# sb17v/GaussianK-SGD

Hardware: AMD Instinct MI355X
Metric: images/sec (whole node) ResNet-50 k=0.1% at 1/2/4/8 MI355X; effective grad compression ratio (higher is better)
Workload: dtype fp32; 1 GPU; model=resnet50, global_batch=512, per_gpu_batch=512, image_size=224, parallelism=dp1, compressor=gaussian, buckets=1, threshold=524288000, planner=threshold, exchange=local, momentum_correction=True, hip_graph=False, f32_matmul=bf16x6

## Files before the change

gaussiank_sgd_amd/ops/conv1x1.py:

```python
from __future__ import annotations

import os
from typing import Callable, Dict, List, Tuple

import torch
import torch.nn as nn
import torch.nn.functional as F

from . import load
from . import streams
from . import weight_prep

_CL = torch.channels_last
_TUNE = os.environ.get("GKSGD_GEMM_TUNE", "1") != "0"
_ENABLED = os.environ.get("GKSGD_FASTCONV", "1") != "0"
_choices: Dict[tuple, tuple] = {}
_OWN = ("hip", "w3", "mat", "wino", "wx6")
_GK_MARGIN = float(os.environ.get("GKSGD_GK_MARGIN", "0.05"))
_BIAS_COLSUM = os.environ.get("GKSGD_CONV_BIAS_COLSUM", "1") != "0"
_timings: Dict[tuple, list] = {}
_WINO = os.environ.get("GKSGD_WINO", "1") != "0"
_FORCE = os.environ.get("GKSGD_CONV_FORCE", "")
_WINO_GRIDS = (0, 1 << 20)
_NT_CFGS = [1, 2, 3, 4, 11, 13, 21, 22, 23, 24, 111, 113, 121, 122, 123, 124, 25, 26, 27, 125, 126, 127,
            211, 212, 213, 214, 221, 222, 223, 224]
_NT_GRIDS = (0, 512, 1 << 20)
_TN_CFGS = [(c, s) for c in (1, 2, 3, 4, 5, 6, 7, 8, 21, 22, 23, 24, 27, 9, 29, 101, 121, 102, 122) for s in (0, 128)]
_NT_CFGS_F32 = [1, 2, 3, 4, 7, 11, 12, 13, 14, 21, 22, 23, 24, 101, 102, 103, 104, 201, 202, 203, 204,
                1001, 1002, 1003, 1004, 1005, 1006, 1007, 1021, 1022, 1101, 1102, 1103]
_TN_CFGS_F32 = [(c, s) for c in (1, 2, 3, 4, 5, 6, 7, 8, 9, 11, 12, 13, 14, 15, 16) for s in (0, 64)]
_TN_SMALL_M = 1 << 17
_TN_SMALL_F32 = [(c, s) for c in (4, 5, 11, 14, 15) for s in (16, 32, 128)]


X6 = 100000
_NT_CFGS_X6 = [c + X6 for c in (1, 2, 3, 4, 5, 6, 7, 12, 13, 101, 102, 103, 104, 105, 106, 107, 202, 203, 1001, 1002, 1003)]
_NT_CFGS_X62 = [2 * X6 + t for t in range(1, 8)] + [3 * X6 + t for t in range(1, 8)]
_F32MM = os.environ.get("GKSGD_F32_MATMUL", "bf16x6")


def set_f32_matmul(mode: str) -> str:
    global _F32MM
    if mode not in ("native", "bf16x6"):
        raise ValueError("f32 matmul mode must be 'native' or 'bf16x6', got %r" % (mode,))
    prev, _F32MM = _F32MM, mode
    return prev


def f32_matmul() -> str:
    return _F32MM


def _x6() -> bool:
    return _F32MM == "bf16x6"


_TN_CFGS_X62 = [(2 * X6 + t, sp) for t in (1, 2, 3, 4, 5, 6, 7, 8) for sp in (0, 64)]


def _tn_cfgs(dt: torch.dtype) -> List[Tuple[int, int]]:
    if dt == torch.float32:
# ... 249 lines not shown


def _lz_kw(lz, rows: bool = False) -> dict:
    _, x, coef, padz, padx = lz
    return dict(lz_x=_rows(x) if rows else x, lz_coef=coef, lz_padz=padz, lz_padx=padx)


def _dgrad(dy: torch.Tensor, w: torch.Tensor, x_shape, s: int, lz=None, plink=None, wp: bool = False) -> torch.Tensor:
    N, C, H, W, K, k, p, OH, OW = _geom(x_shape, w, s)
    g = _g()
    dt = dy.dtype
    xs = torch.empty(x_shape, dtype=dt, device=dy.device, memory_format=_CL)
    kw = _lz_kw(lz, rows=(s == 1 and k == 1)) if lz is not None else {}

    def miopen():
        return torch.ops.aten.convolution_backward(dy, xs, w, None, [s, s], [p, p], [1, 1], False, [0, 0], 1,
                                                   [True, False, False])[0]
    cands = []
    split = []
    dx = None
    if s == 2:
        dx = xs
        z = _zero(dy.device)
        run = lambda c, mb: g.conv_dgrad_s2(dy, w, dx, z, c, mb, **kw)
        cands = [(("hip", c, mb), (lambda c=c, mb=mb: run(c, mb))) for c in _nt_cfgs(dt) for mb in _NT_GRIDS]
    if s == 1:
        dx = xs
        if k == 1:
            DY, DX = _rows(dy), _rows(dx)
            Wt = _lazy(lambda: weight_prep.transposed_1x1(w, wp))
            run = lambda c, mb: g.gemm_nt(DY, Wt(), DX, c, mb, **kw)
            if lz is None:
                split = _splitk_cfgs(dt, N * H * W, C, K)
        else:
            wf = _lazy(lambda: weight_prep.flipped_3x3(w, wp))
            z = _zero(dy.device)
            run = lambda c, mb: g.conv_nt(dy, wf(), dx, z, 1, p, c, mb, **kw)
        cands = [(("hip", c, mb), (lambda c=c, mb=mb: run(c, mb))) for c in _nt_cfgs(dt) for mb in _NT_GRIDS]
        cands += [(("hip", c, mb), (lambda c=c, mb=mb: run(c, mb))) for c in split for mb in _SPLITK_GRIDS]
    if lz is not None:
        cands.append((("mat", 0, 0), lambda: _dgrad(plink.materialize(), w, x_shape, s, wp=wp)))
        ch = _pick(("dgrad", N, C, H, W, K, k, s) + _dkey(dt) + ("lz",), cands)
        if ch[0] == "mat":
            return _dgrad(plink.materialize(), w, x_shape, s, wp=wp)
        run(ch[1], ch[2])
        return dx
    wino = _wino_ok(dt, k, s, K, C) and _wino_shape_fits(N, H, W, C, K)
    if wino:
# ... 8 lines not shown
    run(ch[1], ch[2])
    return dx


_WGRAD_AFTER = os.environ.get("GKSGD_WGRAD_AFTER_DGRAD", "0") == "1"
_SIDE_QROUNDS = int(os.environ.get("GKSGD_WGRAD_SIDE_QROUNDS", "0"))
_FORK_BIAS = os.environ.get("GKSGD_WGRAD_STREAM_BIAS", "0") == "1"
_FORKABLE = tuple(k for k in os.environ.get("GKSGD_WGRAD_STREAM_KINDS", "hip,w3,wino").split(",")
                  if k and (k != "wino" or os.environ.get("GKSGD_WGRAD_STREAM_WINO", "1") == "1"))


def _lazy(make):
    box = []

    def get():
        if not box:
            box.append(make())
        return box[0]
    return get


def _dgrad_key(N, C, H, W, K, k, s, dt) -> tuple:
    wino = _wino_ok(dt, k, s, K, C) and _wino_shape_fits(N, H, W, C, K)
    return ("dgrad", N, C, H, W, K, k, s) + _dkey(dt) + (_wino_tag(K, C) if wino else ())


def _dgrad_bn(dy: torch.Tensor, w: torch.Tensor, x_shape, s: int, link, lz=None, plink=None,
              wp: bool = False) -> torch.Tensor:
    N, C, H, W, K, k, p, OH, OW = _geom(x_shape, w, s)
    kw = _lz_kw(lz, rows=(k == 1)) if lz is not None else {}
    g = _g()
    M = N * H * W
    dt = dy.dtype
    dz = torch.empty(x_shape, dtype=dt, device=dy.device, memory_format=_CL)
    st = torch.empty(2, min(1280, (M + 63) // 64), C, dtype=torch.float32, device=dy.device)
    h, mask, dy2 = link.h, link.mask, link.dy2
    if k == 1:
        DY, DZ = _rows(dy), _rows(dz)
        Wt = _lazy(lambda: weight_prep.transposed_1x1(w, wp))
        H2 = _rows(h)
        D2 = _rows(dy2) if dy2 is not None else None
        run = lambda c, mb: g.gemm_nt(DY, Wt(), DZ, c, mb, st, None, H2, D2, mask, **kw)
        split = _splitk_cfgs(dt, M, C, K) if lz is None else []
    else:
        split = []
        wf = _lazy(lambda: weight_prep.flipped_3x3(w, wp))
        z = _zero(dy.device)
# ... 288 lines not shown
```

gaussiank_sgd_amd/ops/csrc/bindings.cpp:

```cpp
#include <ATen/ATen.h>
#include <c10/core/DeviceGuard.h>
#include <c10/hip/HIPStream.h>
#include <torch/custom_class.h>
#include <torch/library.h>

#include <cstring>
#include <vector>

#include "comm/rccl_engine.h"
#include "kernels/gk_kernels.h"

namespace {

hipStream_t cur_stream(const at::Tensor& t) {
  return c10::hip::getCurrentHIPStream(t.device().index()).stream();
}

void check_dev(const at::Tensor& t, const char* name) {
  TORCH_CHECK(t.is_cuda(), name, " must be a GPU tensor");
  TORCH_CHECK(t.is_contiguous(), name, " must be contiguous");
}

void check_f32(const at::Tensor& t, const char* name) {
  check_dev(t, name);
// ... 1324 lines not shown
void wino_wgrad(at::Tensor x, at::Tensor dy, at::Tensor out, at::Tensor part, int64_t splits) {
  auto cl = [](const at::Tensor& t) {
    return t.is_cuda() && t.scalar_type() == at::kFloat && t.dim() == 4 && t.is_contiguous(at::MemoryFormat::ChannelsLast);
  };
  TORCH_CHECK(cl(x) && cl(dy) && cl(out), "wino_wgrad: x, dy, out must be channels-last fp32 GPU tensors");
  const int64_t N = x.size(0), C = x.size(1), H = x.size(2), W = x.size(3), K = dy.size(1);
  TORCH_CHECK(dy.size(0) == N && dy.size(2) == H && dy.size(3) == W, "wino_wgrad: dy must be [N, K, H, W]");
  TORCH_CHECK(out.size(0) == K && out.size(1) == C && out.size(2) == 3 && out.size(3) == 3,
              "wino_wgrad: out must be [K, C, 3, 3]");
  TORCH_CHECK(C % 64 == 0 && K % 64 == 0, "wino_wgrad: C and K must be multiples of 64");
  TORCH_CHECK(N * ((H + 1) / 2) * ((W + 1) / 2) < (int64_t(1) << 31) && x.numel() * 4 < (int64_t(1) << 31) &&
                  dy.numel() * 4 < (int64_t(1) << 31),
              "wino_wgrad: size out of range (x, dy bytes < 2^31: buffer-descriptor addressing)");
  TORCH_CHECK(part.is_cuda() && part.scalar_type() == at::kFloat && part.is_contiguous() &&
                  part.numel() >= wino_wgrad_ws(N, H, W, C, K, splits),
              "wino_wgrad: workspace too small (wino_wgrad_ws)");
  c10::DeviceGuard guard(x.device());
  gk::wino_wgrad(x.data_ptr<float>(), dy.data_ptr<float>(), part.data_ptr<float>(), out.data_ptr<float>(), (int)N,
                 (int)H, (int)W, (int)C, (int)K, (int)splits, cur_stream(x));
}

void conv_dgrad_s2(at::Tensor dy, at::Tensor w, at::Tensor dx, at::Tensor zero, int64_t cfg, int64_t max_blocks,
                   c10::optional<at::Tensor> lz_x, c10::optional<at::Tensor> lz_coef,
                c10::optional<at::Tensor> lz_padz, c10::optional<at::Tensor> lz_padx) {
  TORCH_CHECK(dy.is_cuda() && is_gemm_dtype(dy) && dy.dim() == 4 && dy.is_contiguous(at::MemoryFormat::ChannelsLast),
              "conv_dgrad_s2: dy must be channels-last bf16 or fp32");
  TORCH_CHECK(w.is_cuda() && w.scalar_type() == dy.scalar_type() && w.dim() == 4 && w.size(0) == dy.size(1) &&
                  w.size(2) == w.size(3) && (w.size(2) == 1 || w.size(2) == 3),
              "conv_dgrad_s2: w must be [K, C, k, k] of dy's dtype, k in {1, 3}");
  TORCH_CHECK(dx.is_cuda() && dx.scalar_type() == dy.scalar_type() && dx.dim() == 4 && dx.size(0) == dy.size(0) &&
                  dx.size(1) == w.size(1) && dx.is_contiguous(at::MemoryFormat::ChannelsLast),
              "conv_dgrad_s2: dx must be channels-last [N, C, H, W] of dy's dtype");
  const bool f32 = dy.scalar_type() == at::kFloat;
  const int64_t N = dy.size(0), K = dy.size(1), OHd = dy.size(2), OWd = dy.size(3);
  const int64_t C = w.size(1), k = w.size(2), H = dx.size(2), W = dx.size(3);
  const int64_t p = k / 2;
  TORCH_CHECK((H + 2 * p - k) / 2 + 1 == OHd && (W + 2 * p - k) / 2 + 1 == OWd, "conv_dgrad_s2: shape mismatch");
  TORCH_CHECK(K % 64 == 0 && C % 64 == 0, "conv_dgrad_s2: channels must be multiples of 64");
  check_zero(zero);
  TORCH_CHECK(N * H * W < (int64_t(1) << 31), "conv_dgrad_s2: too many pixels");
  gk::LazyArgs lzv{};
  const gk::LazyArgs* lz = lazy_args(lz_x, lz_coef, lz_padz, lz_padx, dy, K, &lzv) ? &lzv : nullptr;
  c10::DeviceGuard guard(dy.device());
  const hipStream_t st = cur_stream(dy);
  if (k == 1) {
    const at::Tensor wt = w.reshape({K, C}).t().contiguous();
    const int r = gk::conv_nt_remap(dy.data_ptr(), K, zero.data_ptr(), (int)OHd, (int)OWd, (int)K, (int)OHd,
                                    (int)OWd, 1, 1, wt.data_ptr(), dx.data_ptr(), N * OHd * OWd, (int)C, (int)H, (int)W,
                                    0, 0, 1, f32, (int)cfg, (int)max_blocks, lz, st);
    TORCH_CHECK(r >= 0, "conv_dgrad_s2: the lazy operand's coefficient table does not fit this tile configuration");
    return;
  }
  const at::Tensor wt = w.permute({1, 2, 3, 0}).contiguous();
  for (int a = 0; a < 2; ++a) {
    for (int b = 0; b < 2; ++b) {
      const int64_t OHc = (H - a + 1) / 2, OWc = (W - b + 1) / 2;
      if (OHc <= 0 || OWc <= 0) continue;
      at::Tensor wc = a == 0 ? wt.slice(1, 1, 2) : wt.slice(1, 0, 3, 2).flip({1});
      wc = b == 0 ? wc.slice(2, 1, 2) : wc.slice(2, 0, 3, 2).flip({2});
      wc = wc.contiguous();
      const int r = gk::conv_nt_remap(dy.data_ptr(), K, zero.data_ptr(), (int)OHd, (int)OWd, (int)K, (int)OHc,
                                      (int)OWc, a == 0 ? 1 : 2, b == 0 ? 1 : 2, wc.data_ptr(), dx.data_ptr(),
                                      N * OHc * OWc, (int)C, (int)H, (int)W, a, b, 0, f32, (int)cfg, (int)max_blocks,
                                      lz, st);
      TORCH_CHECK(r >= 0, "conv_dgrad_s2: the lazy operand's coefficient table does not fit this tile configuration");
    }
  }
}

int64_t wgrad3_ws(int64_t N, int64_t H, int64_t W, int64_t C, int64_t K) {
  return gk::wgrad3_ws_floats((int)N, (int)H, (int)W, (int)C, (int)K);
}

void conv3_wgrad(at::Tensor dy, at::Tensor x, at::Tensor out, at::Tensor part, at::Tensor zero) {
  TORCH_CHECK(x.is_cuda() && x.scalar_type() == at::kBFloat16 && x.dim() == 4 &&
                  x.is_contiguous(at::MemoryFormat::ChannelsLast),
              "conv3_wgrad: x must be channels-last bf16 [N, C, H, W]");
  const int64_t N = x.size(0), C = x.size(1), H = x.size(2), W = x.size(3);
  TORCH_CHECK(dy.is_cuda() && dy.scalar_type() == at::kBFloat16 && dy.dim() == 4 && dy.size(0) == N &&
                  dy.size(2) == H && dy.size(3) == W && dy.is_contiguous(at::MemoryFormat::ChannelsLast),
              "conv3_wgrad: dy must be channels-last bf16 [N, K, H, W]");
  const int64_t K = dy.size(1);
  TORCH_CHECK(gk::wgrad3_supported((int)H, (int)W, (int)C, (int)K), "conv3_wgrad: unsupported shape");
  TORCH_CHECK(N * H * W < (int64_t(1) << 31), "conv3_wgrad: too many pixels");
  TORCH_CHECK(out.is_cuda() && out.scalar_type() == at::kFloat && out.dim() == 4 && out.size(0) == K &&
                  out.size(1) == C && out.size(2) == 3 && out.size(3) == 3,
              "conv3_wgrad: out must be fp32 [K, C, 3, 3]");
  TORCH_CHECK(part.is_cuda() && part.scalar_type() == at::kFloat && part.is_contiguous() &&
// ... 528 lines not shown
  m.def("stem_wgrad(Tensor x, Tensor dy, Tensor(a!) out, Tensor(b!) part) -> ()");
  m.def("stem_f32_supported(int H, int W) -> bool", [](int64_t H, int64_t W) { return gk::stem_f32_supported((int)H, (int)W); });
  m.def("stem_f32_fwd(Tensor x, Tensor w, Tensor(a!) y, Tensor(b!)? stats=None) -> int");
  m.def("stem_f32x6_wplanes() -> int", &stem_f32x6_wplanes);
  m.def("stem_f32x6_fwd(Tensor x, Tensor w, Tensor(a!) y, Tensor(b!)? stats, Tensor(c!) wp3) -> int");
  m.def("stem_f32_wgrad_ws(int N) -> int", &stem_f32_wgrad_ws);
  m.def("stem_f32_wgrad(Tensor x, Tensor dy, Tensor(a!) out, Tensor(b!) part, bool x6=False) -> ()");
  m.def("wgrad3_supported(int H, int W, int C, int K) -> bool", [](int64_t H, int64_t W, int64_t C, int64_t K) {
    return gk::wgrad3_supported((int)H, (int)W, (int)C, (int)K);
  });
  m.def("wgrad3_ws(int N, int H, int W, int C, int K) -> int", &wgrad3_ws);
  m.def("conv3_wgrad(Tensor dy, Tensor x, Tensor(a!) out, Tensor(b!) part, Tensor zero) -> ()");
  m.def("wino_weights(Tensor w, Tensor(a!) u, bool flip) -> ()");
  m.def("weight_prep(Tensor table, int ndesc, int total_blocks) -> ()");
  m.def("weight_prep_blocks(int kind, int R, int S) -> int", &weight_prep_blocks);
  m.def("wino_wgrad_ws(int N, int H, int W, int C, int K, int splits=0) -> int", &wino_wgrad_ws);
  m.def("wino_wgrad(Tensor x, Tensor dy, Tensor(a!) out, Tensor(b!) part, int splits=0) -> ()");
  m.def("wino_conv(Tensor x, Tensor u, Tensor(a!) y, int max_blocks=0, Tensor(b!)? stats=None, Tensor? bn_h=None, "
        "Tensor? bn_dy2=None, Tensor? bn_mask=None, int splits=1) -> int");
  m.def("wino_x6_weights(Tensor w, Tensor(a!) u3, bool flip) -> ()");
  m.def("wino_x6_conv(Tensor x, Tensor u3, Tensor(a!) y, int max_blocks=0, Tensor(b!)? stats=None, "
        "Tensor? bn_h=None, Tensor? bn_dy2=None, Tensor? bn_mask=None) -> int");
  m.def("conv_dgrad_s2(Tensor dy, Tensor w, Tensor(a!) dx, Tensor zero, int cfg=0, int max_blocks=0, "
        "Tensor? lz_x=None, Tensor? lz_coef=None, Tensor? lz_padz=None, Tensor? lz_padx=None) -> ()");
  m.def("bn_bwd_lazy_pre(Tensor x, Tensor part, int rows, Tensor? w, Tensor mean, Tensor invstd, "
        "Tensor(a!) dgamma, Tensor(b!) dbeta, Tensor(c!) coef, Tensor(d!) padz, Tensor(e!) padx, "
        "Tensor(f!)? gw_acc=None, Tensor(g!)? gb_acc=None) -> ()");
  m.def("bn_act_backward_lazy(Tensor dy, Tensor? dy2, Tensor? mask, Tensor x, Tensor(a!) dz, Tensor? w, "
        "Tensor mean, Tensor invstd, Tensor(b!) dgamma, Tensor(c!) dbeta, Tensor(d!) ws, bool relu, "
        "Tensor(e!) coef, Tensor(f!) padz, Tensor(g!) padx, Tensor(h!)? gw_acc=None, Tensor(i!)? gb_acc=None) -> ()");
  m.def("bn_lazy_apply(Tensor dz, Tensor x, Tensor(a!) dx, Tensor coef) -> ()");
  m.def("bn_stats_partials(Tensor x, Tensor(a!) ws) -> ()");
  m.def(
      "bn_act_backward_pre_dual(Tensor dz, Tensor x, Tensor(a!) dx, Tensor? w, Tensor mean, Tensor invstd, "
      "Tensor(b!) dgamma, Tensor(c!) dbeta, Tensor part, int rows, Tensor(d!)? gw_acc, Tensor(e!)? gb_acc, Tensor x2, "
      "Tensor(f!) dx2, Tensor? w2, Tensor mean2, Tensor invstd2, Tensor(g!) dgamma2, Tensor(h!) dbeta2, "
      "Tensor(i!) ws2, Tensor(j!)? gw2_acc, Tensor(k!)? gb2_acc) -> ()");
  m.def("bn_act_backward_pre(Tensor dz, Tensor x, Tensor(a!) dx, Tensor? w, Tensor mean, Tensor invstd, "
        "Tensor(b!) dgamma, Tensor(c!) dbeta, Tensor part, int rows, Tensor(d!)? gw_acc=None, "
        "Tensor(e!)? gb_acc=None, Tensor(f!)? fin=None) -> ()");
  m.def("bn_fin_state_bytes(int C) -> int", &bn_fin_state_bytes);
  m.def("attn_supported(int T, int D) -> bool",
        [](int64_t T, int64_t D) { return gk::attn_supported((int)T, (int)D); });
  m.def("attn_fwd(Tensor qkv, Tensor(a!) out, Tensor(b!) lse, int heads, float p, int seed, Tensor? seed_dev=None) -> ()");
  m.def("attn_bwd(Tensor qkv, Tensor out, Tensor dout, Tensor lse, Tensor(a!) delta, Tensor(b!) dqkv, int heads, "
        "float p, int seed, Tensor? seed_dev=None) -> ()");
  m.def("attn_dropout_mask(Tensor(a!) mask, int B, int heads, int T, float p, int seed, Tensor? seed_dev=None) -> ()");
// ... 128 lines not shown
```

gaussiank_sgd_amd/ops/csrc/kernels/gemm.hip:

```cpp
#include "gemm_kern.h"

namespace gk {

static int nt_unit_b16(bool gather, GK_NT_UNIT_ARGS) {
  return gather ? nt_b16_gat(GK_NT_UNIT_PASS) : nt_b16_row(GK_NT_UNIT_PASS);
}

static int nt_unit_f32(bool gather, GK_NT_UNIT_ARGS) {
  const int fam = (cfg / 100000) % 10;
  if (fam == 2 || fam == 3) {
    if (lza || geo.KZ > 1 || geo.RH || (fam == 3) != (geo.b3 != nullptr)) return -2;
    if (gather) {
      const int64_t nimg = M / ((int64_t)geo.OH * geo.OW);
      if (geo.C % 32 != 0 || nimg * geo.H * geo.W * geo.C >= ((int64_t)1 << 31)) return -2;
      return nt_x62_gat(static_cast<const float*>(A), static_cast<const float*>(B), static_cast<float*>(C), M, N, K,
                        cfg % 100000, max_blocks, geo, stats, stats_ld, stats_rows, bb, stream);
    }
    return nt_x62_row(static_cast<const float*>(A), lda, static_cast<const float*>(B), ldb, static_cast<float*>(C),
                      ldc, M, N, K, cfg % 100000, max_blocks, geo.bias, stats, stats_ld, stats_rows, bb, geo.b3, stream);
  }
  const bool x6 = (cfg / 100000) % 10 == 1;
  cfg %= 100000;
  if (x6) return gather ? nt_x6_gat(GK_NT_UNIT_PASS) : nt_x6_row(GK_NT_UNIT_PASS);
  return gather ? nt_f32_gat(GK_NT_UNIT_PASS) : nt_f32_row(GK_NT_UNIT_PASS);
}

static int tn_unit_f32x(bool gather, const float* G, int64_t ldg, const float* X, int64_t ldx, float* W, int64_t ldw,
                        int64_t M, int N, int K, int cfg, int splits, const ConvGeo& geo, const LazyArgs* lza,
                        hipStream_t stream) {
  const int fam = (cfg / 100000) % 10;
  if (fam == 3) return -2;
  if (fam == 2) {
    if (gather || lza) return -2;
    tn_x62_row(G, ldg, X, ldx, W, ldw, M, N, K, cfg % 100000, splits, stream);
  } else if (fam == 1) {
    tn_unit_x6(gather, G, ldg, X, ldx, W, ldw, M, N, K, cfg % 100000, splits, geo, lza, stream);
  } else {
    tn_unit_f32(gather, G, ldg, X, ldx, W, ldw, M, N, K, cfg % 100000, splits, geo, lza, stream);
  }
  return 0;
}

// ... 129 lines not shown
  ConvGeo g{zero, H, W, C, OH, OW, S, P, KW, bias};
  g.b3 = static_cast<const uint16_t*>(b3);
  const int K = KH * KW * C;
  const int SK = (cfg / 10000) % 10;
  const int x6 = cfg / 100000 * 100000;
  if (SK > 1) {
    const int nks = K / 32;
    if (!f32 || lazy || splitk_ws == nullptr || nks % SK != 0 || C % 32 != 0) return -1;
    ConvGeo gz{zero, H, W, C, OH, OW, S, P, KW, nullptr};
    gz.KZ = SK;
    const int r = nt_unit_f32(true, X, C, B, K, splitk_ws, N, M, N, K / SK, x6 + cfg % 10000, max_blocks, gz,
                                           nullptr, 0, 0, BnBwd{}, nullptr, stream);
    if (r < 0) return r;
    return splitk_reduce(splitk_ws, SK, M, N, static_cast<float*>(Y), N, bias, stats, stats_rows, bn, stream);
  }
  const BnBwd bb = bn ? BnBwd{bn->h, bn->dy2, bn->mask} : BnBwd{};
  const int64_t sld = (int64_t)stats_rows * N;
  return f32 ? nt_unit_f32(true, X, C, B, K, Y, N, M, N, K, cfg, max_blocks, g, stats, sld, stats_rows, bb, lazy, stream)
             : nt_unit_b16(true, X, C, B, K, Y, N, M, N, K, cfg, max_blocks, g, stats, sld, stats_rows, bb, nullptr, stream);
}

int conv_nt_remap(const void* X, int64_t ldx, const void* zero, int H, int W, int C, int OH, int OW, int KH, int KW,
                  const void* B, void* Y, int64_t M, int N, int RH, int RW, int RA, int RB, int RZ, bool f32, int cfg,
                  int max_blocks, const LazyArgs* lazy, hipStream_t stream) {
  ConvGeo g{zero, H, W, C, OH, OW, 1, 0, KW, nullptr, RH, RW, RA, RB, RZ};
  const int K = KH * KW * C;
  if (KH * KW == 1) {
    return f32 ? nt_unit_f32(false, X, ldx, B, K, Y, N, M, N, K, cfg, max_blocks, g, nullptr, 0, 0, BnBwd{}, lazy, stream)
               : nt_unit_b16(false, X, ldx, B, K, Y, N, M, N, K, cfg, max_blocks, g, nullptr, 0, 0, BnBwd{}, nullptr, stream);
  }
  return f32 ? nt_unit_f32(true, X, C, B, K, Y, N, M, N, K, cfg, max_blocks, g, nullptr, 0, 0, BnBwd{}, lazy, stream)
             : nt_unit_b16(true, X, C, B, K, Y, N, M, N, K, cfg, max_blocks, g, nullptr, 0, 0, BnBwd{}, nullptr, stream);
}

int gemm_tn_acc(const void* G, int64_t ldg, const void* X, int64_t ldx, float* W, int64_t ldw, int64_t M, int N,
                 int K, bool f32, int cfg, int splits, const LazyArgs* lazy, hipStream_t stream) {
  if (f32)
    return tn_unit_f32x(false, static_cast<const float*>(G), ldg, static_cast<const float*>(X), ldx, W, ldw, M, N, K, cfg,
                           splits, ConvGeo{}, lazy, stream);
  tn_unit_b16(false, G, ldg, X, ldx, W, ldw, M, N, K, cfg, splits, ConvGeo{}, stream);
  return 0;
}

int conv_tn_acc(const void* G, const void* X, const void* zero, int H, int W_, int C, int OH, int OW, int S, int P,
                 int KH, int KW, float* Wout, int64_t M, int N, bool f32, int cfg, int splits, const LazyArgs* lazy,
                 hipStream_t stream) {
  ConvGeo g{zero, H, W_, C, OH, OW, S, P, KW, nullptr};
  const int K = KH * KW * C;
// ... 9 lines not shown
```

gaussiank_sgd_amd/ops/csrc/kernels/gemm_inst.hip:

```cpp
#include "gemm_kern.h"

#ifndef GK_GEMM_UNIT
#error "compile with -DGK_GEMM_UNIT=<unit>"
#endif

namespace gk {

#if GK_GEMM_UNIT == 0
int nt_b16_row(GK_NT_UNIT_ARGS) { return nt_dispatch<false, uint16_t>(GK_NT_UNIT_PASS); }
#elif GK_GEMM_UNIT == 1
int nt_b16_gat(GK_NT_UNIT_ARGS) { return nt_dispatch<true, uint16_t>(GK_NT_UNIT_PASS); }
#elif GK_GEMM_UNIT == 2
int nt_f32_row(GK_NT_UNIT_ARGS) { return nt_dispatch<false, float>(GK_NT_UNIT_PASS); }
#elif GK_GEMM_UNIT == 3
int nt_f32_gat(GK_NT_UNIT_ARGS) { return nt_dispatch<true, float>(GK_NT_UNIT_PASS); }
#elif GK_GEMM_UNIT == 4
void tn_unit_b16(bool gather, const void* G, int64_t ldg, const void* X, int64_t ldx, float* W, int64_t ldw, int64_t M,
                 int N, int K, int cfg, int splits, const ConvGeo& geo, hipStream_t stream) {
  if (gather) tn_dispatch<true>(G, ldg, X, ldx, W, ldw, M, N, K, cfg, splits, geo, stream);
  else tn_dispatch<false>(G, ldg, X, ldx, W, ldw, M, N, K, cfg, splits, geo, stream);
}
void tn_unit_f32(bool gather, const float* G, int64_t ldg, const float* X, int64_t ldx, float* W, int64_t ldw,
                 int64_t M, int N, int K, int cfg, int splits, const ConvGeo& geo, const LazyArgs* lza,
                 hipStream_t stream) {
  if (gather) tn_f32_dispatch<true>(G, ldg, X, ldx, W, ldw, M, N, K, cfg, splits, geo, lza, stream);
  else tn_f32_dispatch<false>(G, ldg, X, ldx, W, ldw, M, N, K, cfg, splits, geo, lza, stream);
}
#elif GK_GEMM_UNIT == 5
int nt_x6_row(GK_NT_UNIT_ARGS) { return nt_dispatch<false, float, true>(GK_NT_UNIT_PASS); }
#elif GK_GEMM_UNIT == 6
int nt_x6_gat(GK_NT_UNIT_ARGS) { return nt_dispatch<true, float, true>(GK_NT_UNIT_PASS); }
#elif GK_GEMM_UNIT == 7
void tn_unit_x6(bool gather, const float* G, int64_t ldg, const float* X, int64_t ldx, float* W, int64_t ldw,
                int64_t M, int N, int K, int cfg, int splits, const ConvGeo& geo, const LazyArgs* lza,
                hipStream_t stream) {
  if (gather) tn_f32_dispatch<true, true>(G, ldg, X, ldx, W, ldw, M, N, K, cfg, splits, geo, lza, stream);
  else tn_f32_dispatch<false, true>(G, ldg, X, ldx, W, ldw, M, N, K, cfg, splits, geo, lza, stream);
}
#elif GK_GEMM_UNIT == 8
int nt_x62_row(const float* A, int64_t lda, const float* B, int64_t ldb, float* C, int64_t ldc, int64_t M, int N, int K,
               int cfg, int max_blocks, const float* bias, float* stats, int64_t stats_ld, int stats_rows,
               const BnBwd& bb, const uint16_t* b3, hipStream_t stream) {
  ConvGeo g{};
  g.b3 = b3;
  return nt_x62_dispatch<false>(A, lda, B, ldb, C, ldc, M, N, K, cfg, max_blocks, bias, stats, stats_ld, stats_rows, bb,
                                g, stream);
}
#elif GK_GEMM_UNIT == 9
void tn_x62_row(const float* G, int64_t ldg, const float* X, int64_t ldx, float* W, int64_t ldw, int64_t M, int N,
                int K, int cfg, int splits, hipStream_t stream) {
  tn_x62_dispatch(G, ldg, X, ldx, W, ldw, M, N, K, cfg, splits, stream);
}
#elif GK_GEMM_UNIT == 10
int nt_x62_gat(const float* A, const float* B, float* C, int64_t M, int N, int K, int cfg, int max_blocks,
               const ConvGeo& geo, float* stats, int64_t stats_ld, int stats_rows, const BnBwd& bb,
               hipStream_t stream) {
  return nt_x62_dispatch<true>(A, geo.C, B, K, C, N, M, N, K, cfg, max_blocks, geo.bias, stats, stats_ld, stats_rows,
                               bb, geo, stream);
}
#else
#error "unknown GK_GEMM_UNIT"
#endif

}
```

gaussiank_sgd_amd/ops/csrc/kernels/gemm_kern.h:

```cpp
#pragma once

#ifndef GK_XCD_REMAP
#define GK_XCD_REMAP 1
#endif
#ifndef GK_X6_SCHED
#define GK_X6_SCHED 1
#endif
#ifndef GK_X6_EXP
#define GK_X6_EXP 0
#endif
#include <hip/hip_runtime.h>

#include <type_traits>

#include "common.h"
#include "gk_kernels.h"
#include "mfma_util.h"
namespace gk {

constexpr int kMaxTaps = 4;

struct ConvGeo {
  const void* zero;
  int H, W, C, OH, OW, S, P, KW;
// ... 9 lines not shown
  const uint8_t* mask;
};

struct LazyA {
  const void* x;
  const float* coef;
  const void* padz;
  const void* padx;
  int C;
};

#define GK_NT_UNIT_ARGS                                                                                      \
  const void *A, int64_t lda, const void *B, int64_t ldb, void *C, int64_t ldc, int64_t M, int N, int K, int cfg, \
      int max_blocks, const ConvGeo &geo, float *stats, int64_t stats_ld, int stats_rows, const BnBwd &bb,      \
      const LazyArgs *lza, hipStream_t stream
#define GK_NT_UNIT_PASS A, lda, B, ldb, C, ldc, M, N, K, cfg, max_blocks, geo, stats, stats_ld, stats_rows, bb, lza, stream
int nt_b16_row(GK_NT_UNIT_ARGS);
int nt_b16_gat(GK_NT_UNIT_ARGS);
int nt_f32_row(GK_NT_UNIT_ARGS);
int nt_f32_gat(GK_NT_UNIT_ARGS);
int nt_x6_row(GK_NT_UNIT_ARGS);
int nt_x6_gat(GK_NT_UNIT_ARGS);
int nt_x62_row(const float* A, int64_t lda, const float* B, int64_t ldb, float* C, int64_t ldc, int64_t M, int N, int K,
               int cfg, int max_blocks, const float* bias, float* stats, int64_t stats_ld, int stats_rows,
               const BnBwd& bb, const uint16_t* b3, hipStream_t stream);
int nt_x62_gat(const float* A, const float* B, float* C, int64_t M, int N, int K, int cfg, int max_blocks,
               const ConvGeo& geo, float* stats, int64_t stats_ld, int stats_rows, const BnBwd& bb,
               hipStream_t stream);
void tn_x62_row(const float* G, int64_t ldg, const float* X, int64_t ldx, float* W, int64_t ldw, int64_t M, int N,
                int K, int cfg, int splits, hipStream_t stream);
void tn_unit_x6(bool gather, const float* G, int64_t ldg, const float* X, int64_t ldx, float* W, int64_t ldw,
                int64_t M, int N, int K, int cfg, int splits, const ConvGeo& geo, const LazyArgs* lza,
                hipStream_t stream);
void tn_unit_b16(bool gather, const void* G, int64_t ldg, const void* X, int64_t ldx, float* W, int64_t ldw, int64_t M,
                 int N, int K, int cfg, int splits, const ConvGeo& geo, hipStream_t stream);
void tn_unit_f32(bool gather, const float* G, int64_t ldg, const float* X, int64_t ldx, float* W, int64_t ldw,
                 int64_t M, int N, int K, int cfg, int splits, const ConvGeo& geo, const LazyArgs* lza,
                 hipStream_t stream);

namespace {

__device__ __forceinline__ int swz(int r) { return (r >> 1) & 7; }

__device__ __forceinline__ void xcd_remap2(int& bx, int& by) {
  const int gx = (int)gridDim.x, gy = (int)gridDim.y, G = gx * gy;
  bx = (int)blockIdx.x;
  by = (int)blockIdx.y;
  if (!GK_XCD_REMAP || (G & 7) != 0 || G < 16) return;
// ... 505 lines not shown
      }
    }
    if (pf) stage_advance();
    st3 = st2;
    st2 = st1;
    st1 = 0;
    if (++ks == nk) {
      ks = 0;
      const int64_t mbase = mt * Cfg::BM;
      mt += gridDim.x;
      const bool full = mbase + Cfg::BM <= M;
      const bool odd = fq & 1;
#pragma unroll
      for (int ms = 0; ms < MSB; ++ms) {
        const int64_t m = mbase + wm * Cfg::WTM + ms * 16 + fr;
        const bool live = full || m < M;
        int64_t orow = m;
        int zr = 0, zc = 0;
        if (geo.RH) {
          const uint32_t ohw = (uint32_t)(geo.OH * geo.OW);
          const uint32_t mu = (uint32_t)(m < M ? m : M - 1);
          const uint32_t ni = mu / ohw, rem = mu - ni * ohw;
          const uint32_t oh = rem / (uint32_t)geo.OW, ow = rem - oh * (uint32_t)geo.OW;
          orow = ((int64_t)ni * geo.RH + 2 * oh + geo.RA) * geo.RW + 2 * ow + geo.RB;
          zr = (int)(2 * oh + 1) < geo.RH;
          zc = (int)(2 * ow + 1) < geo.RW;
        }
        if constexpr (F32) {
          f32x4 ehv[4], ed2[4];
          uint32_t ebits[4];
          if constexpr (PRE) {
            const int slot = ms % PMS;
#pragma unroll
            for (int ns = 0; ns < 4; ++ns) {
              ehv[ns] = pre_h[slot][ns];
              ed2[ns] = pre_d[slot][ns];
              ebits[ns] = pre_b[slot][ns];
            }
            if (ms + PMS < MSB) bn_row_load(mbase, ms + PMS, pre_h[slot], pre_d[slot], pre_b[slot]);
          } else if (bnb) {
#pragma unroll
            for (int ns = 0; ns < 4; ++ns) {
              ehv[ns] = ed2[ns] = f32x4{0.f, 0.f, 0.f, 0.f};
              ebits[ns] = 0u;
            }
            if (live) {
#pragma unroll
// ... 991 lines not shown
      if (pc >= 0 && pc != Cfg::PRA + p) continue;
      const int cid = tid + Cfg::THREADS * p;
      const int r = cid >> 2;
      const int off = r * 64 + (((cid & 3) ^ x62_swz(r)) << 4);
      if constexpr (P3) {
        *reinterpret_cast<u32x4*>(sb + off) = rb3[q][p][0];
        *reinterpret_cast<u32x4*>(sb + Cfg::PB + off) = rb3[q][p][1];
        *reinterpret_cast<u32x4*>(sb + 2 * Cfg::PB + off) = rb3[q][p][2];
      } else {
        bf16x8 h, m, l;
        split3x8(rb[q][p][0], rb[q][p][1], h, m, l);
        *reinterpret_cast<bf16x8*>(sb + off) = h;
        *reinterpret_cast<bf16x8*>(sb + Cfg::PB + off) = m;
        *reinterpret_cast<bf16x8*>(sb + 2 * Cfg::PB + off) = l;
      }
    }
  };

  f32x4 acc[4][4];
#pragma unroll
  for (int a = 0; a < 4; ++a)
#pragma unroll
    for (int b = 0; b < 4; ++b) acc[a][b] = f32x4{0.f, 0.f, 0.f, 0.f};
  float ssum[4][4], ssq[4][4], bia[BNB ? 1 : 4][4];
#pragma unroll
  for (int a = 0; a < 4; ++a)
#pragma unroll
    for (int b = 0; b < 4; ++b) {
      ssum[a][b] = ssq[a][b] = 0.f;
      if constexpr (!BNB) bia[a][b] = bias ? bias[n0 + wn * 64 + a * 16 + fq * 4 + b] : 0.f;
    }

  auto epilogue = [&](int64_t mt) __attribute__((always_inline)) {
    const int64_t mbase = mt * Cfg::BM;
    constexpr int EH = BNB ? 1 : 4;
#pragma unroll
    for (int ms = 0; ms < 4; ++ms) {
      const int64_t m = mbase + wm * 64 + ms * 16 + fr;
      const bool live = m < M;
#pragma unroll
      for (int nh = 0; nh < 4; nh += EH) {
      f32x4 ehv[EH], ed2[EH];
      uint32_t ebits[EH];
      if constexpr (BNB) {
#pragma unroll
        for (int e = 0; e < EH; ++e) {
          ehv[e] = ed2[e] = f32x4{0.f, 0.f, 0.f, 0.f};
          ebits[e] = 0u;
        }
        if (live) {
#pragma unroll
          for (int e = 0; e < EH; ++e) {
            const int n = n0 + wn * 64 + (nh + e) * 16 + fq * 4;
            ehv[e] = *reinterpret_cast<const f32x4*>(static_cast<const float*>(bb.h) + m * ldc + n);
            if (bb.dy2) ed2[e] = *reinterpret_cast<const f32x4*>(static_cast<const float*>(bb.dy2) + m * ldc + n);
            ebits[e] = bb.mask ? (uint32_t)bb.mask[m * (Ntot >> 2) + (n >> 2)] : 0xfu;
          }
        }
      }
#pragma unroll
      for (int e = 0; e < EH; ++e) {
        const int ns = nh + e;
// ... 1 lines not shown
        f32x4 v = acc[ms][ns];
        acc[ms][ns] = f32x4{0.f, 0.f, 0.f, 0.f};
        if constexpr (!BNB) {
#pragma unroll
          for (int r = 0; r < 4; ++r) v[r] += bia[ns][r];
        }
        if constexpr (BNB) {
#pragma unroll
          for (int r = 0; r < 4; ++r) {
            const float dz = (ebits[e] >> r) & 1u ? v[r] + ed2[e][r] : 0.f;
            v[r] = dz;
            ssum[ns][r] += dz;
            ssq[ns][r] = fmaf(dz, ehv[e][r], ssq[ns][r]);
          }
        } else {
          if (stats && live) {
#pragma unroll
            for (int r = 0; r < 4; ++r) {
              ssum[ns][r] += v[r];
              ssq[ns][r] = fmaf(v[r], v[r], ssq[ns][r]);
            }
          }
        }
        if (live) *reinterpret_cast<f32x4*>(C + m * ldc + n) = v;
      }
      }
    }
  };

  using I0 = std::integral_constant<int, 0>;
  using I1 = std::integral_constant<int, (NPF > 1 ? 1 : 0)>;
  issue_loads(I0{});
  split_write(0, I0{});
  if (T_ > 1) issue_loads(I1{});
  if (NPF > 1 && T_ > 2) issue_loads(I0{});
  __syncthreads();
  int ks = 0;
  int64_t mt = bx;
  auto slice = [&](int t, auto PAR) __attribute__((always_inline)) {
    constexpr int par = decltype(PAR)::value;
    using SN = std::integral_constant<int, (NPF > 1 ? (par ^ 1) : 0)>;
    const int cur = par;
    const char* st = smem + cur * Cfg::STAGE;
    const char* pa = st;
    const char* pb = st + 3 * Cfg::PA;
    auto frag = [&](const char* plane, int row) __attribute__((always_inline)) -> bf16x8 {
      return *reinterpret_cast<const bf16x8*>(plane + row * 64 + ((fq ^ x62_swz(row)) << 4));
    };
// ... 468 lines not shown
```

gaussiank_sgd_amd/ops/csrc/kernels/gk_kernels.h:

```cpp
#pragma once

#include <hip/hip_runtime.h>
#include <stddef.h>
#include <stdint.h>

namespace gk {

enum Mode : int {
  kModeGaussian = 0,
  kModeRedSync = 1,
  kModeRedSyncTrim = 2,
  kModeTopK = 3,
  kModeRandomK = 4,
  kModeThreshold = 5,
  kModeDGC = 6,
  kModeGaussianCal = 7,
};

constexpr int kCalFallback = 16;
constexpr int kOverflowExact = 17;

constexpr int kMaxCand = 16;
constexpr int kRecHdr = 4;
constexpr int kMaxCountBlocks = 1024;
// ... 216 lines not shown
  const uint8_t* mask;
};
struct LazyArgs {
  const void* x;
  const float* coef;
  const void* padz;
  const void* padx;
  int C;
};
int gemm_nt(const void* A, int64_t lda, const void* B, int64_t ldb, void* C, int64_t ldc, int64_t M, int N, int K,
            bool f32, int cfg, int max_blocks, float* stats, int stats_rows, const float* bias, const BnBwdArgs* bn,
            const LazyArgs* lazy, hipStream_t stream, float* splitk_ws = nullptr, const void* b3 = nullptr);
int splitk_reduce(const float* ws, int S, int64_t M, int N, float* C, int64_t ldc, const float* bias, float* stats,
                  int stats_rows, const BnBwdArgs* bn, hipStream_t stream);
int gemm_tn_acc(const void* G, int64_t ldg, const void* X, int64_t ldx, float* W, int64_t ldw, int64_t M, int N,
                 int K, bool f32, int cfg, int splits, const LazyArgs* lazy, hipStream_t stream);
int conv_nt(const void* X, const void* zero, int H, int W, int C, int OH, int OW, int S, int P, int KH, int KW,
            const void* B, void* Y, int64_t M, int N, bool f32, int cfg, int max_blocks, float* stats, int stats_rows,
            const float* bias, const BnBwdArgs* bn, const LazyArgs* lazy, hipStream_t stream,
            float* splitk_ws = nullptr, const void* b3 = nullptr);
void split3_rows(const float* src, int64_t ld, void* dst, int64_t R, int S, hipStream_t stream);
int conv_nt_remap(const void* X, int64_t ldx, const void* zero, int H, int W, int C, int OH, int OW, int KH, int KW,
                  const void* B, void* Y, int64_t M, int N, int RH, int RW, int RA, int RB, int RZ, bool f32, int cfg,
                  int max_blocks, const LazyArgs* lazy, hipStream_t stream);
int conv_tn_acc(const void* G, const void* X, const void* zero, int H, int W, int C, int OH, int OW, int S, int P,
                 int KH, int KW, float* Wout, int64_t M, int N, bool f32, int cfg, int splits, const LazyArgs* lazy,
                 hipStream_t stream);
bool stem_f32_supported(int H, int W);
int stem_f32_wgrad_blocks(int N);
int stem_f32x6_wplanes();
int stem_f32x6_forward(const float* x, int N, int H, int W, const float* w, int64_t s0, int64_t s1, int64_t s2,
                       int64_t s3, uint16_t* wp3, float* y, float* stats, int stats_rows, hipStream_t stream);
int stem_f32_forward(const float* x, int N, int H, int W, const float* w, int64_t s0, int64_t s1, int64_t s2,
                     int64_t s3, float* y, float* stats, int stats_rows, hipStream_t stream);
void stem_f32_wgrad(const float* x, const float* dy, int N, int H, int W, float* part, float* out, int64_t s0,
                    int64_t s1, int64_t s2, int64_t s3, bool x6, hipStream_t stream);
void wino_weights(const float* w, float* u, int Co, int Ci, int flip, hipStream_t stream);
enum PrepKind : int32_t { kPrepWino = 0, kPrepWinoFlip = 1, kPrepT32 = 2, kPrepT16 = 3, kPrepWinoX6 = 4,
                          kPrepWinoX6Flip = 5 };
struct PrepDesc {
  const void* src;
  void* dst;
  int64_t ld_in, ld_out;
  int64_t block_begin;
  int32_t kind, R, S, tiles_s;
};
static_assert(sizeof(PrepDesc) == 56, "PrepDesc layout is packed by ops/weight_prep.py");
// ... 91 lines not shown
```

gaussiank_sgd_amd/ops/weight_prep.py:

```python
from __future__ import annotations

import contextlib
import os
import struct
import threading
from typing import Callable, Dict, List, Optional, Tuple

import torch

KIND_WINO, KIND_WINO_FLIP, KIND_T32, KIND_T16, KIND_WINO_X6, KIND_WINO_X6_FLIP = 0, 1, 2, 3, 4, 5
_DESC = struct.Struct("<QQqqqiiii")
_MAX_DESCS = 512
_tls = threading.local()
ENABLED = os.environ.get("GKSGD_WEIGHT_PREP", "1") != "0"


def _ops():
    return torch.ops.gksgd


class _Entry:
    __slots__ = ("src", "dst", "descs", "ready")

    def __init__(self, src: torch.Tensor, dst: torch.Tensor, descs: List[tuple]):
# ... 146 lines not shown


def flipped_3x3(w: torch.Tensor, persistent: bool) -> torch.Tensor:
    K, C = w.shape[0], w.shape[1]

    def make():
        return torch.empty((C, K, 3, 3), dtype=w.dtype, device=w.device, memory_format=torch.channels_last)

    def fill(out):
        out.copy_(w.flip(2, 3).transpose(0, 1))
    p = current()
    if p is None or not persistent or w.dtype not in (torch.float32, torch.bfloat16) or \
            not w.is_contiguous(memory_format=torch.channels_last):
        out = make()
        fill(out)
        return out
    kind = KIND_T32 if w.dtype == torch.float32 else KIND_T16
    es = w.element_size()

    def descs(out):
        return [(kind, w.data_ptr() + (8 - t) * C * es, out.data_ptr() + t * K * es, 9 * C, 9 * K, K, C)
                for t in range(9)]
    return p.acquire(_key("f3", w), w, make, descs, fill)
```

Before: 5152 images/s.

## Enable bf16x6 register-staged kernels and cached class filters for stride-2 dgrad

Stride-2 dgrad can now use the register-staged bf16x6 GEMM family. The epilogue gains row remapping, using fast magic-number division, and sibling zero-fill, so those kernels accept remapped output geometry. Per-parity class filters for the 3x3 and 1x1 stride-2 weights are precomputed and cached through the weight-prep machinery, which removes the per-call permute, slice and contiguous copies. This adds more autotune candidates and a per-call bf16 presplit for family-3 configs, plus more complex epilogue indexing that could raise register pressure.

After: 5149 images/s, median of 2. No clear change (-0.0%).

```diff
diff --git a/gaussiank_sgd_amd/ops/conv1x1.py b/gaussiank_sgd_amd/ops/conv1x1.py
--- a/gaussiank_sgd_amd/ops/conv1x1.py
+++ b/gaussiank_sgd_amd/ops/conv1x1.py
@@ -37,6 +37,8 @@
 _NT_CFGS_X6 = [c + X6 for c in (1, 2, 3, 4, 5, 6, 7, 12, 13, 101, 102, 103, 104, 105, 106, 107, 202, 203, 1001, 1002, 1003)]
 _NT_CFGS_X62 = [2 * X6 + t for t in range(1, 8)] + [3 * X6 + t for t in range(1, 8)]
 _F32MM = os.environ.get("GKSGD_F32_MATMUL", "bf16x6")
+_S2_X62 = os.environ.get("GKSGD_DGRAD_S2_X62", "1") != "0"
+_S2_PREP = os.environ.get("GKSGD_DGRAD_S2_PREP", "1") != "0"
 
 
 def set_f32_matmul(mode: str) -> str:
@@ -332,8 +334,10 @@
     if s == 2:
         dx = xs
         z = _zero(dy.device)
-        run = lambda c, mb: g.conv_dgrad_s2(dy, w, dx, z, c, mb, **kw)
-        cands = [(("hip", c, mb), (lambda c=c, mb=mb: run(c, mb))) for c in _nt_cfgs(dt) for mb in _NT_GRIDS]
+        wc = _lazy(lambda: weight_prep.dgrad_s2_filters(w, wp)) if _S2_PREP else (lambda: None)
+        run = lambda c, mb: g.conv_dgrad_s2(dy, w, dx, z, c, mb, wcls=wc(), **kw)
+        cfgs = [c for c in _nt_cfgs(dt) if _S2_X62 or c not in _NT_CFGS_X62]
+        cands = [(("hip", c, mb), (lambda c=c, mb=mb: run(c, mb))) for c in cfgs for mb in _NT_GRIDS]
     if s == 1:
         dx = xs
         if k == 1:
@@ -388,7 +392,9 @@
 
 def _dgrad_key(N, C, H, W, K, k, s, dt) -> tuple:
     wino = _wino_ok(dt, k, s, K, C) and _wino_shape_fits(N, H, W, C, K)
-    return ("dgrad", N, C, H, W, K, k, s) + _dkey(dt) + (_wino_tag(K, C) if wino else ())
+    nox62 = s == 2 and not _S2_X62 and dt == torch.float32 and _x6()
+    return ("dgrad", N, C, H, W, K, k, s) + _dkey(dt) + (_wino_tag(K, C) if wino else ()) + \
+        (("nox62",) if nox62 else ())
 
 
 def _dgrad_bn(dy: torch.Tensor, w: torch.Tensor, x_shape, s: int, link, lz=None, plink=None,
diff --git a/gaussiank_sgd_amd/ops/csrc/bindings.cpp b/gaussiank_sgd_amd/ops/csrc/bindings.cpp
--- a/gaussiank_sgd_amd/ops/csrc/bindings.cpp
+++ b/gaussiank_sgd_amd/ops/csrc/bindings.cpp
@@ -1370,7 +1370,8 @@
 
 void conv_dgrad_s2(at::Tensor dy, at::Tensor w, at::Tensor dx, at::Tensor zero, int64_t cfg, int64_t max_blocks,
                    c10::optional<at::Tensor> lz_x, c10::optional<at::Tensor> lz_coef,
-                c10::optional<at::Tensor> lz_padz, c10::optional<at::Tensor> lz_padx) {
+                   c10::optional<at::Tensor> lz_padz, c10::optional<at::Tensor> lz_padx,
+                   c10::optional<at::Tensor> wcls) {
   TORCH_CHECK(dy.is_cuda() && is_gemm_dtype(dy) && dy.dim() == 4 && dy.is_contiguous(at::MemoryFormat::ChannelsLast),
               "conv_dgrad_s2: dy must be channels-last bf16 or fp32");
   TORCH_CHECK(w.is_cuda() && w.scalar_type() == dy.scalar_type() && w.dim() == 4 && w.size(0) == dy.size(1) &&
@@ -1391,27 +1392,60 @@
   const gk::LazyArgs* lz = lazy_args(lz_x, lz_coef, lz_padz, lz_padx, dy, K, &lzv) ? &lzv : nullptr;
   c10::DeviceGuard guard(dy.device());
   const hipStream_t st = cur_stream(dy);
+  if (wcls.has_value()) {
+    TORCH_CHECK(wcls->is_cuda() && wcls->scalar_type() == w.scalar_type() && wcls->is_contiguous() &&
+                    wcls->numel() == k * k * C * K,
+                "conv_dgrad_s2: wcls must hold the k * k * C * K class-filter elements of w's dtype");
+  }
+  const bool fam3 = (cfg / 100000) % 10 == 3;
+  TORCH_CHECK(!fam3 || f32, "conv_dgrad_s2: cfg family 3 takes fp32 operands");
+  auto presplit = [&](const void* wc, int64_t S) {
+    at::Tensor b3 = at::empty({C, 3 * S}, w.options().dtype(at::kBFloat16));
+    gk::split3_rows(static_cast<const float*>(wc), S, b3.data_ptr(), C, (int)S, st);
+    return b3;
+  };
+  const char* refused_x62 = "conv_dgrad_s2: the register-staged bf16x6 kernels (cfg digit 200000/300000) take no "
+                            "lazy operand or split-K";
+  const char* refused = "conv_dgrad_s2: the lazy operand's coefficient table does not fit this tile configuration";
   if (k == 1) {
-    const at::Tensor wt = w.reshape({K, C}).t().contiguous();
+    const at::Tensor wt = wcls.has_value() ? *wcls : w.reshape({K, C}).t().contiguous();
+    at::Tensor b3;
+    if (fam3) b3 = presplit(wt.data_ptr(), K);
     const int r = gk::conv_nt_remap(dy.data_ptr(), K, zero.data_ptr(), (int)OHd, (int)OWd, (int)K, (int)OHd,
                                     (int)OWd, 1, 1, wt.data_ptr(), dx.data_ptr(), N * OHd * OWd, (int)C, (int)H, (int)W,
-                                    0, 0, 1, f32, (int)cfg, (int)max_blocks, lz, st);
-    TORCH_CHECK(r >= 0, "conv_dgrad_s2: the lazy operand's coefficient table does not fit this tile configuration");
+                                    0, 0, 1, f32, (int)cfg, (int)max_blocks, lz, st,
+                                    b3.defined() ? b3.data_ptr() : nullptr);
+    TORCH_CHECK(r != -2, refused_x62);
+    TORCH_CHECK(r >= 0, refused);
     return;
   }
-  const at::Tensor wt = w.permute({1, 2, 3, 0}).contiguous();
+  at::Tensor wt;
+  if (!wcls.has_value()) wt = w.permute({1, 2, 3, 0}).contiguous();
+  int64_t woff = 0;
   for (int a = 0; a < 2; ++a) {
     for (int b = 0; b < 2; ++b) {
+      const int KHc = a == 0 ? 1 : 2, KWc = b == 0 ? 1 : 2;
+      const int64_t wn = (int64_t)KHc * KWc * C * K;
+      const int64_t wo = woff;
+      woff += wn;
       const int64_t OHc = (H - a + 1) / 2, OWc = (W - b + 1) / 2;
       if (OHc <= 0 || OWc <= 0) continue;
-      at::Tensor wc = a == 0 ? wt.slice(1, 1, 2) : wt.slice(1, 0, 3, 2).flip({1});
-      wc = b == 0 ? wc.slice(2, 1, 2) : wc.slice(2, 0, 3, 2).flip({2});
-      wc = wc.contiguous();
+      at::Tensor wc;
+      if (wcls.has_value()) {
+        wc = wcls->view({-1}).narrow(0, wo, wn);
+      } else {
+        wc = a == 0 ? wt.slice(1, 1, 2) : wt.slice(1, 0, 3, 2).flip({1});
+        wc = b == 0 ? wc.slice(2, 1, 2) : wc.slice(2, 0, 3, 2).flip({2});
+        wc = wc.contiguous();
+      }
+      at::Tensor b3;
+      if (fam3) b3 = presplit(wc.data_ptr(), (int64_t)KHc * KWc * K);
       const int r = gk::conv_nt_remap(dy.data_ptr(), K, zero.data_ptr(), (int)OHd, (int)OWd, (int)K, (int)OHc,
-                                      (int)OWc, a == 0 ? 1 : 2, b == 0 ? 1 : 2, wc.data_ptr(), dx.data_ptr(),
+                                      (int)OWc, KHc, KWc, wc.data_ptr(), dx.data_ptr(),
                                       N * OHc * OWc, (int)C, (int)H, (int)W, a, b, 0, f32, (int)cfg, (int)max_blocks,
-                                      lz, st);
-      TORCH_CHECK(r >= 0, "conv_dgrad_s2: the lazy operand's coefficient table does not fit this tile configuration");
+                                      lz, st, b3.defined() ? b3.data_ptr() : nullptr);
+      TORCH_CHECK(r != -2, refused_x62);
+      TORCH_CHECK(r >= 0, refused);
     }
   }
 }
@@ -1986,7 +2020,7 @@
   m.def("wino_x6_conv(Tensor x, Tensor u3, Tensor(a!) y, int max_blocks=0, Tensor(b!)? stats=None, "
         "Tensor? bn_h=None, Tensor? bn_dy2=None, Tensor? bn_mask=None) -> int");
   m.def("conv_dgrad_s2(Tensor dy, Tensor w, Tensor(a!) dx, Tensor zero, int cfg=0, int max_blocks=0, "
-        "Tensor? lz_x=None, Tensor? lz_coef=None, Tensor? lz_padz=None, Tensor? lz_padx=None) -> ()");
+        "Tensor? lz_x=None, Tensor? lz_coef=None, Tensor? lz_padz=None, Tensor? lz_padx=None, Tensor? wcls=None) -> ()");
   m.def("bn_bwd_lazy_pre(Tensor x, Tensor part, int rows, Tensor? w, Tensor mean, Tensor invstd, "
         "Tensor(a!) dgamma, Tensor(b!) dbeta, Tensor(c!) coef, Tensor(d!) padz, Tensor(e!) padx, "
         "Tensor(f!)? gw_acc=None, Tensor(g!)? gb_acc=None) -> ()");
diff --git a/gaussiank_sgd_amd/ops/csrc/kernels/gemm.hip b/gaussiank_sgd_amd/ops/csrc/kernels/gemm.hip
--- a/gaussiank_sgd_amd/ops/csrc/kernels/gemm.hip
+++ b/gaussiank_sgd_amd/ops/csrc/kernels/gemm.hip
@@ -9,7 +9,7 @@
 static int nt_unit_f32(bool gather, GK_NT_UNIT_ARGS) {
   const int fam = (cfg / 100000) % 10;
   if (fam == 2 || fam == 3) {
-    if (lza || geo.KZ > 1 || geo.RH || (fam == 3) != (geo.b3 != nullptr)) return -2;
+    if (lza || geo.KZ > 1 || (geo.RH && bb.h) || (fam == 3) != (geo.b3 != nullptr)) return -2;
     if (gather) {
       const int64_t nimg = M / ((int64_t)geo.OH * geo.OW);
       if (geo.C % 32 != 0 || nimg * geo.H * geo.W * geo.C >= ((int64_t)1 << 31)) return -2;
@@ -17,7 +17,7 @@
                         cfg % 100000, max_blocks, geo, stats, stats_ld, stats_rows, bb, stream);
     }
     return nt_x62_row(static_cast<const float*>(A), lda, static_cast<const float*>(B), ldb, static_cast<float*>(C),
-                      ldc, M, N, K, cfg % 100000, max_blocks, geo.bias, stats, stats_ld, stats_rows, bb, geo.b3, stream);
+                      ldc, M, N, K, cfg % 100000, max_blocks, geo, stats, stats_ld, stats_rows, bb, stream);
   }
   const bool x6 = (cfg / 100000) % 10 == 1;
   cfg %= 100000;
@@ -193,8 +193,9 @@
 
 int conv_nt_remap(const void* X, int64_t ldx, const void* zero, int H, int W, int C, int OH, int OW, int KH, int KW,
                   const void* B, void* Y, int64_t M, int N, int RH, int RW, int RA, int RB, int RZ, bool f32, int cfg,
-                  int max_blocks, const LazyArgs* lazy, hipStream_t stream) {
+                  int max_blocks, const LazyArgs* lazy, hipStream_t stream, const void* b3) {
   ConvGeo g{zero, H, W, C, OH, OW, 1, 0, KW, nullptr, RH, RW, RA, RB, RZ};
+  g.b3 = static_cast<const uint16_t*>(b3);
   const int K = KH * KW * C;
   if (KH * KW == 1) {
     return f32 ? nt_unit_f32(false, X, ldx, B, K, Y, N, M, N, K, cfg, max_blocks, g, nullptr, 0, 0, BnBwd{}, lazy, stream)
diff --git a/gaussiank_sgd_amd/ops/csrc/kernels/gemm_inst.hip b/gaussiank_sgd_amd/ops/csrc/kernels/gemm_inst.hip
--- a/gaussiank_sgd_amd/ops/csrc/kernels/gemm_inst.hip
+++ b/gaussiank_sgd_amd/ops/csrc/kernels/gemm_inst.hip
@@ -39,12 +39,10 @@
 }
 #elif GK_GEMM_UNIT == 8
 int nt_x62_row(const float* A, int64_t lda, const float* B, int64_t ldb, float* C, int64_t ldc, int64_t M, int N, int K,
-               int cfg, int max_blocks, const float* bias, float* stats, int64_t stats_ld, int stats_rows,
-               const BnBwd& bb, const uint16_t* b3, hipStream_t stream) {
-  ConvGeo g{};
-  g.b3 = b3;
-  return nt_x62_dispatch<false>(A, lda, B, ldb, C, ldc, M, N, K, cfg, max_blocks, bias, stats, stats_ld, stats_rows, bb,
-                                g, stream);
+               int cfg, int max_blocks, const ConvGeo& geo, float* stats, int64_t stats_ld, int stats_rows,
+               const BnBwd& bb, hipStream_t stream) {
+  return nt_x62_dispatch<false>(A, lda, B, ldb, C, ldc, M, N, K, cfg, max_blocks, geo.bias, stats, stats_ld, stats_rows,
+                                bb, geo, stream);
 }
 #elif GK_GEMM_UNIT == 9
 void tn_x62_row(const float* G, int64_t ldg, const float* X, int64_t ldx, float* W, int64_t ldw, int64_t M, int N,
diff --git a/gaussiank_sgd_amd/ops/csrc/kernels/gemm_kern.h b/gaussiank_sgd_amd/ops/csrc/kernels/gemm_kern.h
--- a/gaussiank_sgd_amd/ops/csrc/kernels/gemm_kern.h
+++ b/gaussiank_sgd_amd/ops/csrc/kernels/gemm_kern.h
@@ -55,8 +55,8 @@
 int nt_x6_row(GK_NT_UNIT_ARGS);
 int nt_x6_gat(GK_NT_UNIT_ARGS);
 int nt_x62_row(const float* A, int64_t lda, const float* B, int64_t ldb, float* C, int64_t ldc, int64_t M, int N, int K,
-               int cfg, int max_blocks, const float* bias, float* stats, int64_t stats_ld, int stats_rows,
-               const BnBwd& bb, const uint16_t* b3, hipStream_t stream);
+               int cfg, int max_blocks, const ConvGeo& geo, float* stats, int64_t stats_ld, int stats_rows,
+               const BnBwd& bb, hipStream_t stream);
 int nt_x62_gat(const float* A, const float* B, float* C, int64_t M, int N, int K, int cfg, int max_blocks,
                const ConvGeo& geo, float* stats, int64_t stats_ld, int stats_rows, const BnBwd& bb,
                hipStream_t stream);
@@ -608,7 +608,7 @@
           const uint32_t mu = (uint32_t)(m < M ? m : M - 1);
           const uint32_t ni = mu / ohw, rem = mu - ni * ohw;
           const uint32_t oh = rem / (uint32_t)geo.OW, ow = rem - oh * (uint32_t)geo.OW;
-          orow = ((int64_t)ni * geo.RH + 2 * oh + geo.RA) * geo.RW + 2 * ow + geo.RB;
+        orow = (int64_t)((ni * (uint32_t)geo.RH + 2 * oh + (uint32_t)geo.RA) * (uint32_t)geo.RW + 2 * ow + (uint32_t)geo.RB);
           zr = (int)(2 * oh + 1) < geo.RH;
           zc = (int)(2 * ow + 1) < geo.RW;
         }
@@ -1646,22 +1646,50 @@
   for (int a = 0; a < 4; ++a)
 #pragma unroll
     for (int b = 0; b < 4; ++b) acc[a][b] = f32x4{0.f, 0.f, 0.f, 0.f};
-  float ssum[4][4], ssq[4][4], bia[BNB ? 1 : 4][4];
+  float ssum[4][4], ssq[4][4];
 #pragma unroll
   for (int a = 0; a < 4; ++a)
 #pragma unroll
-    for (int b = 0; b < 4; ++b) {
-      ssum[a][b] = ssq[a][b] = 0.f;
-      if constexpr (!BNB) bia[a][b] = bias ? bias[n0 + wn * 64 + a * 16 + fq * 4 + b] : 0.f;
-    }
-
+    for (int b = 0; b < 4; ++b) ssum[a][b] = ssq[a][b] = 0.f;
+
+  uint32_t rq_hw = 0u, rq_w = 0u;
+  if (!BNB && geo.RH) {
+    rq_hw = (uint32_t)__builtin_amdgcn_readfirstlane((int)(0xffffffffu / (uint32_t)(geo.OH * geo.OW)));
+    rq_w = (uint32_t)__builtin_amdgcn_readfirstlane((int)(0xffffffffu / (uint32_t)geo.OW));
+  }
   auto epilogue = [&](int64_t mt) __attribute__((always_inline)) {
     const int64_t mbase = mt * Cfg::BM;
     constexpr int EH = BNB ? 1 : 4;
+    f32x4 bia[BNB ? 1 : 4];
+    if constexpr (!BNB) {
+#pragma unroll
+      for (int ns = 0; ns < 4; ++ns)
+#pragma unroll
+        for (int r = 0; r < 4; ++r) bia[ns][r] = bias ? bias[n0 + wn * 64 + ns * 16 + fq * 4 + r] : 0.f;
+    }
 #pragma unroll
     for (int ms = 0; ms < 4; ++ms) {
       const int64_t m = mbase + wm * 64 + ms * 16 + fr;
       const bool live = m < M;
+      int drow = 0, zsib = 0;
+      if (!BNB && geo.RH) {
+        const uint32_t ohw = (uint32_t)(geo.OH * geo.OW);
+        const uint32_t mu = (uint32_t)(live ? m : M - 1);
+        uint32_t ni = __umulhi(mu, rq_hw), rem = mu - ni * ohw;
+        if (rem >= ohw) {
+          ++ni;
+          rem -= ohw;
+        }
+        uint32_t oh = __umulhi(rem, rq_w), ow = rem - oh * (uint32_t)geo.OW;
+        if (ow >= (uint32_t)geo.OW) {
+          ++oh;
+          ow -= (uint32_t)geo.OW;
+        }
+        drow = (int)((ni * (uint32_t)geo.RH + 2 * oh + (uint32_t)geo.RA) * (uint32_t)geo.RW + 2 * ow +
+                     (uint32_t)geo.RB - mu);
+        if (geo.RZ && live) zsib = (int)((int)(2 * ow + 1) < geo.RW) | ((int)((int)(2 * oh + 1) < geo.RH) << 1);
+      }
+      const int64_t doff = (int64_t)drow * ldc;
 #pragma unroll
       for (int nh = 0; nh < 4; nh += EH) {
       f32x4 ehv[EH], ed2[EH];
@@ -1709,8 +1737,18 @@
             }
           }
         }
-        if (live) *reinterpret_cast<f32x4*>(C + m * ldc + n) = v;
-      }
+        if (live) *reinterpret_cast<f32x4*>(C + m * ldc + n + doff) = v;
+      }
+      }
+      if (zsib) {
+        float* zp = C + m * ldc + (n0 + wn * 64 + fq * 4) + doff;
+#pragma unroll
+        for (int ns = 0; ns < 4; ++ns) {
+          const f32x4 z = acc[ms][ns];
+          if (zsib & 1) *reinterpret_cast<f32x4*>(zp + ldc + ns * 16) = z;
+          if (zsib & 2) *reinterpret_cast<f32x4*>(zp + geo.RW * ldc + ns * 16) = z;
+          if (zsib == 3) *reinterpret_cast<f32x4*>(zp + (geo.RW + 1) * ldc + ns * 16) = z;
+        }
       }
     }
   };
diff --git a/gaussiank_sgd_amd/ops/csrc/kernels/gk_kernels.h b/gaussiank_sgd_amd/ops/csrc/kernels/gk_kernels.h
--- a/gaussiank_sgd_amd/ops/csrc/kernels/gk_kernels.h
+++ b/gaussiank_sgd_amd/ops/csrc/kernels/gk_kernels.h
@@ -262,7 +262,7 @@
 void split3_rows(const float* src, int64_t ld, void* dst, int64_t R, int S, hipStream_t stream);
 int conv_nt_remap(const void* X, int64_t ldx, const void* zero, int H, int W, int C, int OH, int OW, int KH, int KW,
                   const void* B, void* Y, int64_t M, int N, int RH, int RW, int RA, int RB, int RZ, bool f32, int cfg,
-                  int max_blocks, const LazyArgs* lazy, hipStream_t stream);
+                  int max_blocks, const LazyArgs* lazy, hipStream_t stream, const void* b3 = nullptr);
 int conv_tn_acc(const void* G, const void* X, const void* zero, int H, int W, int C, int OH, int OW, int S, int P,
                  int KH, int KW, float* Wout, int64_t M, int N, bool f32, int cfg, int splits, const LazyArgs* lazy,
                  hipStream_t stream);
diff --git a/gaussiank_sgd_amd/ops/weight_prep.py b/gaussiank_sgd_amd/ops/weight_prep.py
--- a/gaussiank_sgd_amd/ops/weight_prep.py
+++ b/gaussiank_sgd_amd/ops/weight_prep.py
@@ -192,3 +192,46 @@
         return [(kind, w.data_ptr() + (8 - t) * C * es, out.data_ptr() + t * K * es, 9 * C, 9 * K, K, C)
                 for t in range(9)]
     return p.acquire(_key("f3", w), w, make, descs, fill)
+
+
+def _s2_classes():
+    taps = ((1,), (2, 0))
+    return [(taps[a], taps[b]) for a in (0, 1) for b in (0, 1)]
+
+
+def dgrad_s2_filters(w: torch.Tensor, persistent: bool) -> torch.Tensor:
+    K, C, k = w.shape[0], w.shape[1], w.shape[2]
+    if k == 1:
+        return transposed_1x1(w, persistent)
+
+    def make():
+        return torch.empty(9 * C * K, dtype=w.dtype, device=w.device)
+
+    def fill(out):
+        wt = w.permute(1, 2, 3, 0)
+        off = 0
+        for khs, kws in _s2_classes():
+            wc = wt[:, 1:2] if len(khs) == 1 else wt[:, 0:3:2].flip(1)
+            wc = wc[:, :, 1:2] if len(kws) == 1 else wc[:, :, 0:3:2].flip(2)
+            out[off:off + wc.numel()].view(wc.shape).copy_(wc)
+            off += wc.numel()
+    p = current()
+    if p is None or not persistent or w.dtype not in (torch.float32, torch.bfloat16) or \
+            not w.is_contiguous(memory_format=torch.channels_last):
+        out = make()
+        fill(out)
+        return out
+    kind = KIND_T32 if w.dtype == torch.float32 else KIND_T16
+    es = w.element_size()
+
+    def descs(out):
+        d, off = [], 0
+        for khs, kws in _s2_classes():
+            nt = len(khs) * len(kws)
+            for j, kh in enumerate(khs):
+                for i, kw in enumerate(kws):
+                    d.append((kind, w.data_ptr() + (kh * 3 + kw) * C * es,
+                              out.data_ptr() + (off + (j * len(kws) + i) * K) * es, 9 * C, nt * K, K, C))
+            off += nt * C * K
+        return d
+    return p.acquire(_key("s2", w), w, make, descs, fill)
```
